# DavidPeicho/cuda-pathtracer

Measured on AMD Instinct MI355X. Metric: Msamples/sec at 1920x1080, 4 spp, indoor.obj, higher is better.
Workload: dtype f32

## Files before the change

### cuda-pathtracer_amd/csrc/pt_device.h

```cpp
#pragma once

#include <hip/hip_runtime.h>
#include <stdint.h>

#include "pt_round.h"

namespace ptamd {

struct f3 { float x, y, z; };

#define PT_DEV __device__ __forceinline__
#define PT_HD __host__ __device__ __forceinline__

PT_HD f3 mk3(float x, float y, float z) { f3 r; r.x = x; r.y = y; r.z = z; return r; }
PT_HD f3 mk3(float s) { return mk3(s, s, s); }
PT_HD f3 operator+(f3 a, f3 b) { return mk3(a.x + b.x, a.y + b.y, a.z + b.z); }
PT_HD f3 operator+(f3 a, float b) { return mk3(a.x + b, a.y + b, a.z + b); }
PT_HD f3 operator-(f3 a, f3 b) { return mk3(a.x - b.x, a.y - b.y, a.z - b.z); }
PT_HD f3 operator-(f3 a, float b) { return mk3(a.x - b, a.y - b, a.z - b); }
PT_HD f3 operator-(f3 a) { return mk3(-a.x, -a.y, -a.z); }
PT_HD f3 operator*(f3 a, f3 b) { return mk3(a.x * b.x, a.y * b.y, a.z * b.z); }
PT_HD f3 operator*(f3 a, float b) { return mk3(a.x * b, a.y * b, a.z * b); }
PT_HD f3 operator*(float b, f3 a) { return mk3(b * a.x, b * a.y, b * a.z); }
PT_HD f3 operator/(f3 a, f3 b) { return mk3(a.x / b.x, a.y / b.y, a.z / b.z); }
PT_HD f3 operator/(f3 a, float b) { return mk3(a.x / b, a.y / b, a.z / b); }
PT_HD f3 operator/(float b, f3 a) { return mk3(b / a.x, b / a.y, b / a.z); }
PT_HD float dot(f3 a, f3 b) { return a.x * b.x + a.y * b.y + a.z * b.z; }
PT_HD f3 cross(f3 a, f3 b) { return mk3(a.y * b.z - a.z * b.y, a.z * b.x - a.x * b.z, a.x * b.y - a.y * b.x); }
PT_DEV f3 normalize(f3 v) { float inv_len = 1.0f / __builtin_sqrtf(dot(v, v)); return v * inv_len; }

#ifndef PT_SHORT_MATH
#define PT_SHORT_MATH 1
#endif
PT_DEV float rcp_exact_in_range(float x)
{
  const float y0 = __builtin_amdgcn_rcpf(x);
  const float e0 = __builtin_fmaf(-x, y0, 1.0f);
  const float y1 = __builtin_fmaf(e0, y0, y0);
  const float r1 = __builtin_fmaf(-x, y1, 1.0f);
  const float q1 = __builtin_fmaf(r1, y1, y1);
  const float r2 = __builtin_fmaf(-x, q1, 1.0f);
  return __builtin_fmaf(r2, y1, q1);
}
PT_DEV float sqrt_exact_in_range(float x)
{
  float s = __builtin_amdgcn_sqrtf(x);
  const float sd = __uint_as_float(__float_as_uint(s) - 1u), su = __uint_as_float(__float_as_uint(s) + 1u);
  const float rd = __builtin_fmaf(-sd, s, x), ru = __builtin_fmaf(-su, s, x);
  s = rd <= 0.0f ? sd : s;
  s = ru > 0.0f ? su : s;
  return s;
}
PT_DEV bool wave_all(bool c) { return __builtin_amdgcn_ballot_w64(!c) == 0ull; }
PT_DEV f3 normalize_hot(f3 v)
{
  const float d = dot(v, v);
  float inv_len;
  if (PT_SHORT_MATH && wave_all(d >= 0x1p-96f && d < __builtin_inff())) inv_len = rcp_exact_in_range(sqrt_exact_in_range(d));
  else inv_len = 1.0f / __builtin_sqrtf(d);
  return v * inv_len;
}
PT_DEV float rcp_hot(float x)
{
  if (PT_SHORT_MATH && wave_all(x >= 0x1p-95f && x <= 0x1p125f)) return rcp_exact_in_range(x);
  return 1.0f / x;
}
PT_DEV float sqrt_checked(float x)
{
  if (PT_SHORT_MATH && wave_all(!(x < 0x1p-96f) || x == 0.0f)) return sqrt_exact_in_range(x);
  return __builtin_sqrtf(x);
}
PT_DEV float sqrt_hot(float x) { return PT_SHORT_MATH ? sqrt_exact_in_range(x) : __builtin_sqrtf(x); }
PT_DEV f3 reflect(f3 i, f3 n) { return i - (2.0f * n) * dot(n, i); }
PT_DEV f3 mix(f3 x, f3 y, float a) { return (x * (1.0f - a)) + y * a; }
PT_HD float clamp01(float f) { float m = f < 1.0f ? f : 1.0f; return 0.0f > m ? 0.0f : m; }

PT_DEV uint32_t f_as_u(float f) { return __float_as_uint(f); }
PT_DEV float u_as_f(uint32_t u) { return __uint_as_float(u); }


PT_DEV void pt_sincosf(float x, float& s, float& c)
{
  const float two_over_pi = 0x1.45f306p-1f;
  const float pio2_hi = 0x1.921fb6p+0f;
  const float pio2_lo = -0x1.777a5cp-25f;
  float k = __builtin_rintf(x * two_over_pi);
  float r = __builtin_fmaf(-k, pio2_hi, x);
  r = __builtin_fmaf(-k, pio2_lo, r);
  float r2 = r * r;
  float ps = __builtin_fmaf(__builtin_fmaf(-1.9515295891e-4f, r2, 8.3321608736e-3f), r2, -1.6666654611e-1f);
  float sn = __builtin_fmaf(r * r2, ps, r);
  float pc = __builtin_fmaf(__builtin_fmaf(2.443315711809948e-5f, r2, -1.388731625493765e-3f), r2, 4.166664568298827e-2f);
  float cs = __builtin_fmaf(r2 * r2, pc, __builtin_fmaf(-0.5f, r2, 1.0f));
  int q = (int)k & 3;
  float so = (q & 1) ? cs : sn;
  float co = (q & 1) ? sn : cs;
  if (q == 1 || q == 2) co = -co;
  if (q >= 2) so = -so;
  s = so;
  c = co;
}

__constant__ double kPowLog[9] = { 1.0 / 17.0, 1.0 / 15.0, 1.0 / 13.0, 1.0 / 11.0, 1.0 / 9.0, 1.0 / 7.0, 1.0 / 5.0, 1.0 / 3.0, 1.0 };
__constant__ double kPowExp[14] = { 1.0 / 6227020800.0, 1.0 / 479001600.0, 1.0 / 39916800.0, 1.0 / 3628800.0,
                                    1.0 / 362880.0, 1.0 / 40320.0, 1.0 / 5040.0, 1.0 / 720.0, 1.0 / 120.0,
                                    1.0 / 24.0, 1.0 / 6.0, 0.5, 1.0, 1.0 };

#ifndef __HIP_DEVICE_COMPILE__
static constexpr double kPowLogHost[9] = { 1.0 / 17.0, 1.0 / 15.0, 1.0 / 13.0, 1.0 / 11.0, 1.0 / 9.0, 1.0 / 7.0, 1.0 / 5.0, 1.0 / 3.0, 1.0 };
static constexpr double kPowExpHost[14] = { 1.0 / 6227020800.0, 1.0 / 479001600.0, 1.0 / 39916800.0, 1.0 / 3628800.0,
                                            1.0 / 362880.0, 1.0 / 40320.0, 1.0 / 5040.0, 1.0 / 720.0, 1.0 / 120.0,
                                            1.0 / 24.0, 1.0 / 6.0, 0.5, 1.0, 1.0 };
#define kPowLog kPowLogHost
#define kPowExp kPowExpHost
#define __double_as_longlong(x) __builtin_bit_cast(long long, (double)(x))
#define __longlong_as_double(x) __builtin_bit_cast(double, (long long)(x))
#endif

#ifdef __HIP_DEVICE_COMPILE__
__host__ __device__ __noinline__ float pt_powf(float xf, float yf)
#else
static __host__ __device__ __noinline__ float pt_powf(float xf, float yf)
#endif
{
  if (yf == 0.0f || xf == 1.0f) return 1.0f;
  if (xf != xf || yf != yf) return __builtin_nanf("");
  double x = (double)xf, y = (double)yf;
  bool negate = false;
  if (xf < 0.0f) {
    if (__builtin_floorf(yf) != yf) return __builtin_nanf("");
    float h = __builtin_fabsf(yf) * 0.5f;
    negate = __builtin_floorf(h) != h;
    x = -x;
  }
  double res;
  const double inf = __builtin_inf();
  if (x == 0.0) {
    res = y > 0.0 ? 0.0 : inf;
  } else if (x == inf) {
    res = y > 0.0 ? inf : 0.0;
  } else if (y == inf || y == -inf) {
    res = ((x > 1.0) == (y > 0.0)) ? inf : 0.0;
  } else {
    uint64_t b = (uint64_t)__double_as_longlong(x);
    int e = (int)((b >> 52) & 0x7ff) - 1023;
    double m = __longlong_as_double((long long)((b & 0x000fffffffffffffULL) | 0x3ff0000000000000ULL));
    if (m > 0x1.6a09e667f3bcdp+0) { m *= 0.5; e += 1; }
    double s = (m - 1.0) / (m + 1.0);
    double s2 = s * s;
    double p = kPowLog[0];
#pragma unroll
    for (int i = 1; i < 8; ++i) p = __builtin_fma(p, s2, kPowLog[i]);
    double lnm = 2.0 * s * __builtin_fma(p, s2, kPowLog[8]);
    double log2x = (double)e + lnm * 0x1.71547652b82fep+0;
    double z = y * log2x;
    if (z > 1100.0) {
      res = inf;
    } else if (z < -1100.0) {
      res = 0.0;
    } else {
      double n = __builtin_rint(z);
      double t = (z - n) * 0x1.62e42fefa39efp-1;
      double q = kPowExp[0];
#pragma unroll
      for (int i = 1; i < 14; ++i) q = __builtin_fma(q, t, kPowExp[i]);
      int ni = (int)n;
      int n1 = ni / 2, n2 = ni - n1;
      double s1 = __longlong_as_double((long long)((uint64_t)(n1 + 1023) << 52));
      double s2b = __longlong_as_double((long long)((uint64_t)(n2 + 1023) << 52));
      res = q * s1 * s2b;
    }
  }
  return (float)(negate ? -res : res);
}
#ifndef __HIP_DEVICE_COMPILE__
#undef kPowLog
#undef kPowExp
#undef __double_as_longlong
#undef __longlong_as_double
#endif

PT_HD uint32_t pt_f2u(float v)
{
  if (!(v > 0.0f)) return 0u;
  if (v >= 4294967296.0f) return 0xffffffffu;
  return (uint32_t)v;
}


PT_HD f3 uncharted_tonemap(f3 x)
{
  const float A = 0.15f, B = 0.50f, C = 0.10f, D = 0.20f, E = 0.02f, F = 0.30f;
  return ((x * (A * x + C * B) + D * E) / (x * (A * x + B) + D * F)) - E / F;
}

PT_HD f3 exposure(f3 color)
{
  const float exposure_bias = 2.0f;
  const f3 curr = uncharted_tonemap(exposure_bias * color);
  const f3 W = mk3(11.2f);
  const f3 white_scale = 1.0f / uncharted_tonemap(W);
  return curr * white_scale;
}

PT_HD f3 post_process(uint32_t id, f3 c)
{
  if (id == 1) {
    const float gray = (float)((double)c.x * 0.3 + (double)c.y * 0.59 + (double)c.z * 0.11);
    return mk3(gray, gray, gray);
  }
  if (id == 2)
    return mk3((float)((double)c.x * 0.393 + (double)c.y * 0.769 + (double)c.z * 0.189),
               (float)((double)c.x * 0.349 + (double)c.y * 0.686 + (double)c.z * 0.168),
               (float)((double)c.x * 0.272 + (double)c.y * 0.534 + (double)c.z * 0.131));
  if (id == 3)
    return mk3((float)(1.0 - (double)c.x), (float)(1.0 - (double)c.y), (float)(1.0 - (double)c.z));
  return c;
}

PT_HD uint32_t gamma_byte_exact(float x)
{
  return pt_f2u(pt_powf(x, 1.0f / 2.2f) * 255.0f) & 0xffu;
}
PT_HD uint32_t gamma_value_exact(float x) { return pt_f2u(pt_powf(x, 1.0f / 2.2f) * 255.0f); }

template <typename TablePtr>
PT_DEV uint32_t gamma_byte(float x, TablePtr T)
{
  if (!(x < T[256])) return gamma_byte_exact(x);
  if (!(x > 0.0f)) return 0u;
  const float est = __builtin_amdgcn_exp2f(__builtin_amdgcn_logf(x) * (1.0f / 2.2f)) * 255.0f;
  int k = (int)est;
  k = k < 0 ? 0 : (k > 255 ? 255 : k);
  k = x < T[k] ? k - 1 : k;
  k = x >= T[k + 1] ? k + 1 : k;
  return (uint32_t)k;
}

template <typename TablePtr>
PT_HD uint32_t output_pixel(f3 rad, uint32_t post_id, bool use_table, TablePtr T)
{
  rad = exposure(rad);
#ifdef __HIP_DEVICE_COMPILE__
  if (use_table) return gamma_byte(rad.x, T) | (gamma_byte(rad.y, T) << 8) | (gamma_byte(rad.z, T) << 16);
#endif
  const float g = 1.0f / 2.2f;
  rad = mk3(pt_powf(rad.x, g), pt_powf(rad.y, g), pt_powf(rad.z, g));
  rad = post_process(post_id, rad);
  return (pt_f2u(rad.x * 255.0f) & 0xffu) | ((pt_f2u(rad.y * 255.0f) & 0xffu) << 8) | ((pt_f2u(rad.z * 255.0f) & 0xffu) << 16);
}


struct Xorwow { uint32_t v0, v1, v2, v3, v4, d; };

PT_DEV uint32_t wang_hash(uint32_t a)
{
  a = (a ^ 61u) ^ (a >> 16);
  a = a + (a << 3);
  a = a ^ (a >> 4);
  a = a * 0x27d4eb2du;
  a = a ^ (a >> 15);
  return a;
}

PT_DEV void xorwow_init(Xorwow& st, uint32_t seed)
{
  uint32_t s0 = seed ^ 0xaad26b49u;
  uint32_t s1 = 0xf7dcefddu;
  uint32_t t0 = 1099087573u * s0;
  uint32_t t1 = 2591861531u * s1;
  st.v0 = 123456789u + t0;
  st.v1 = 362436069u ^ t0;
  st.v2 = 521288629u + t1;
  st.v3 = 88675123u ^ t1;
  st.v4 = 5783321u + t0;
  st.d = 6615241u + t1 + t0;
}

PT_HD float xorwow_uniform(Xorwow& st)
{
  uint32_t t = st.v0 ^ (st.v0 >> 2);
  st.v0 = st.v1; st.v1 = st.v2; st.v2 = st.v3; st.v3 = st.v4;
  st.v4 = (st.v4 ^ (st.v4 << 4)) ^ (t ^ (t << 1));
  st.d += 362437u;
  uint32_t x = st.v4 + st.d;
  return (float)x * 2.3283064e-10f + (2.3283064e-10f / 2.0f);
}


PT_HD float max3(f3 v) { return __builtin_fmaxf(v.x, __builtin_fmaxf(v.y, v.z)); }

template <class Rcp>
PT_HD bool miss_tail_iteration(f3 env, int max_bounces, f3& acc, f3& thr, uint32_t& bk, float& r1, Xorwow& rng, Rcp rcp)
{
  acc = acc + env * thr;
  const float pmax = max3(thr);
  if (r1 > pmax && (bk & 0xffffu) > 1u) return true;
  thr = thr * rcp(pmax);
  ++bk;
  if ((int)(bk & 0xffffu) >= max_bounces) return true;
  r1 = xorwow_uniform(rng);
  return false;
}

PT_HD bool miss_tail_is_closed(f3 thr) { return max3(thr) == 1.0f; }
PT_HD uint32_t miss_tail_count(uint32_t b, int max_bounces) { const int n = max_bounces - (int)b; return n > 1 ? (uint32_t)n : 1u; }
template <class Rcp>
PT_HD uint32_t miss_tail_finish(f3 env, int max_bounces, f3& acc, f3& thr, uint32_t& bk, float& r1, Xorwow& rng, Rcp rcp)
{
  uint32_t futile = 0;
  while (!miss_tail_is_closed(thr)) {
    if (miss_tail_iteration(env, max_bounces, acc, thr, bk, r1, rng, rcp)) return futile;
    ++futile;
  }
  const f3 e = env * thr;
  const uint32_t n = miss_tail_count(bk & 0xffffu, max_bounces);
  for (uint32_t i = 0; i < n; ++i) acc = acc + e;
  return futile + n - 1u;
}


struct TexDesc { int32_t w, h, nb_chan; uint32_t pad; uint64_t offset; };

#define PT_HEAD_STRIDE 64u
#ifndef PT_TILE_W_LOG2
#define PT_TILE_W_LOG2 3u
#endif
#define PT_TILE_W (1u << PT_TILE_W_LOG2)
#define PT_TILE_H (64u >> PT_TILE_W_LOG2)
struct KParams {
  const float4* nodes;
  const float4* tris_bvh;
  const float4* tris_brute;
  const float4* shade;
  const int4* materials;
  const float4* lights;
  const TexDesc* textures;
  const float* texels;
  const float4* cubemap;
  uint32_t cubemap_size;
  uint32_t n_faces, n_lights, n_nodes, n_bvh_tris;
  f3 cam_pos, cam_p0, cam_u, cam_v;
  float focus_dist, aperture;
  uint32_t width, height, row_begin, row_end;
  uint32_t hash_seed;
  float frame_nb_f;
  float frame_nb_inv;
  int32_t is_static;
  int32_t bounces;
  uint32_t post_id;
  float* tfb;
  uint32_t* surface;
  uint32_t tfb_row0;
  uint32_t tfb_reset;
  uint32_t surf_row0;
  unsigned long long* stats;
  unsigned long long* error_flag;
  union { uint32_t* tile_counter; uint32_t* adaptive; };
  uint32_t* tile_heads;
  uint32_t n_static;
  uint32_t tiles_x, n_tiles, tiles_per_ticket;
  uint32_t refill_min;
  uint32_t sample_count, frame_nb0;
  float* samples_out;
  float4* pool;
  uint32_t pool_lds_offset;
  uint32_t round_min, round_div;
  uint32_t round_div_m16;
  uint32_t walk_min;
  uint32_t small_det;
  uint32_t env_uniform;
  float env_r, env_g, env_b;
  const float* gamma_table;
  const float4* nodes4;
  uint32_t n_nodes4;
  uint32_t stack_lds_entries, stack_spill_entries;
  uint32_t ilv_ranks, ilv_rank, ilv_rows;
  uint32_t y_limit;
  uint32_t treelet_nodes;
  uint2* stack_spill;
  uint32_t walk_min4;
  uint32_t wide8;
  uint32_t far_table[16];
  uint32_t xcd_regions;
  uint32_t brute_walk;
  unsigned long long* timeline;
  uint32_t round_form;
  uint32_t round_defer;
};
#define PT_ROUND_GENERIC 1u
#define PT_ROUND_FLAT 2u
#define PT_ROUND_SKIP 4u
#define PT_ROUND_DEFER 8u
#define PT_ROUND_TIGHT 16u
inline bool round_form_tight(uint32_t round_form, uint32_t small_det, bool knob)
{
  const uint32_t needs = PT_ROUND_FLAT | PT_ROUND_SKIP | PT_ROUND_DEFER;
  return knob && small_det != 0u && (round_form & needs) == needs;
}
#define PT_SKIP_ENTRY_BYTES 32u

#define PT_RS_PLAIN 0
#define PT_RS_STATS 1
#define PT_RS_STAMPS 2
#define PT_RS_BRUTE 3
#define PT_RS_WIDE8 4
#define PT_RS_WIDE4Q 5
#define PT_RS_GENERIC 6
#define PT_RS_LIST 7
#define PT_RS_FLAT 8
#define PT_RS_FLAT_SKIP 9
#define PT_RS_PLAIN_SKIP 10
#define PT_RS_FLAT_SKIP_DEFER 11
#define PT_RS_PLAIN_SKIP_DEFER 12
#define PT_RS_STATS_DEFER 13
#define PT_RS_FLAT_SKIP_TIGHT 14
#define PT_RS_FORMS 15

struct RestartTraits {
  bool stats;
  bool stamps;
  bool brute;
  int wide;
  bool list;
  bool lean;
  bool flat;
  bool skip;
  bool defer;
  bool tight;
  int reports;
  bool resident, streamed, contracted;
};
constexpr RestartTraits kRestartForms[] = {
  { false, false, false, 0, false, true,  false, false, false, false, PT_RS_PLAIN,      true,  true,  true },
  { true,  false, false, 0, false, false, false, false, false, false, PT_RS_STATS,      true,  true,  false },
  { false, true,  false, 0, false, false, false, false, false, false, PT_RS_STAMPS,     true,  true,  false },
  { false, false, true,  0, false, false, false, false, false, false, PT_RS_BRUTE,      true,  true,  true },
  { false, false, false, 1, false, false, false, false, false, false, PT_RS_WIDE8,      false, true,  false },
  { false, false, false, 2, false, false, false, false, false, false, PT_RS_WIDE4Q,     false, true,  false },
  { false, false, false, 0, false, false, false, false, false, false, PT_RS_GENERIC,    true,  false, true },
  { false, false, false, 0, true,  false, false, false, false, false, PT_RS_LIST,       true,  true,  false },
  { false, false, false, 0, false, true,  true,  false, false, false, PT_RS_FLAT,       true,  false, false },
  { false, false, false, 0, false, true,  true,  true,  false, false, PT_RS_FLAT_SKIP,  true,  false, false },
  { false, false, false, 0, false, true,  false, true,  false, false, PT_RS_PLAIN_SKIP, true,  false, false },
  { false, false, false, 0, false, true,  true,  true,  true,  false, PT_RS_FLAT_SKIP,  true,  false, false },
  { false, false, false, 0, false, true,  false, true,  true,  false, PT_RS_PLAIN_SKIP, true,  false, false },
  { true,  false, false, 0, false, false, false, false, true,  false, PT_RS_STATS,      true,  false, false },
  { false, false, false, 0, false, true,  true,  true,  true,  true,  PT_RS_FLAT_SKIP,  true,  false, false },
};
static_assert(sizeof kRestartForms / sizeof kRestartForms[0] == PT_RS_FORMS, "one row per PT_RS_* number");
constexpr RestartTraits restart_traits(int variant) { return kRestartForms[variant]; }

inline bool restart_shipped_launch(const KParams& p)
{
  return p.is_static && p.pool_lds_offset && !p.xcd_regions && p.ilv_ranks <= 1u && !(p.round_form & PT_ROUND_GENERIC);
}

struct RestartForm { int variant; bool lds_resident; };
inline RestartForm restart_select(bool lds_resident, bool stats, bool list, bool contracted, const KParams* p)
{
  const auto full = [contracted](int variant) { return contracted ? PT_RS_PLAIN : variant; };
  if (list && !contracted) return { PT_RS_LIST, lds_resident };
  const bool defers = p && lds_resident && !contracted && (p->round_form & PT_ROUND_DEFER) && (p->round_form & PT_ROUND_SKIP) && !p->brute_walk && !p->timeline &&
                      restart_shipped_launch(*p);
  if (stats) return { defers ? PT_RS_STATS_DEFER : full(PT_RS_STATS), lds_resident };
  if (p && p->brute_walk) return { PT_RS_BRUTE, lds_resident };
  if (p && p->timeline) return { full(PT_RS_STAMPS), lds_resident };
  if (!lds_resident && p && p->wide8) return { full(p->wide8 == 2u ? PT_RS_WIDE4Q : PT_RS_WIDE8), false };
  if (!lds_resident) return { PT_RS_PLAIN, false };
  if (p && !restart_shipped_launch(*p)) return { PT_RS_GENERIC, true };
  if (defers && (p->round_form & PT_ROUND_FLAT) && (p->round_form & PT_ROUND_TIGHT)) return { PT_RS_FLAT_SKIP_TIGHT, true };
  if (defers) return { (p->round_form & PT_ROUND_FLAT) ? PT_RS_FLAT_SKIP_DEFER : PT_RS_PLAIN_SKIP_DEFER, true };
  if (p && (p->round_form & PT_ROUND_SKIP) && !contracted) return { (p->round_form & PT_ROUND_FLAT) ? PT_RS_FLAT_SKIP : PT_RS_PLAIN_SKIP, true };
  if (p && (p->round_form & PT_ROUND_FLAT)) return { full(PT_RS_FLAT), true };
  return { PT_RS_PLAIN, true };
}
#define PT_POOL_LDS_BYTES 2304u

struct Hit {
  f3 normal;
  f3 diffuse_col;
  float dist;
  float specular_col;
  float ior;
  int light;
  float emission;
};

}
```

### cuda-pathtracer_amd/csrc/pt_kernels.hip

```cpp
#include "pt_device.h"
#include "pt_launch.h"
#include "pt_adaptive.h"

#include <utility>

#if defined(PT_FMA_BUILD) || defined(PT_TIGHT_BUILD)
#define PT_SIDE_UNIT 1
#endif

#ifndef PT_SIDE_UNIT
#include "pt_denoise.h"
#endif

namespace ptamd {

#ifndef PT_TILE_THREADS
#define PT_TILE_THREADS 512
#endif
#ifndef PT_TILE_WAVES_PER_EU
#define PT_TILE_WAVES_PER_EU 6
#endif
#ifndef PT_SP_THREADS
#define PT_SP_THREADS 768
#endif
// ... 1596 lines not shown
      const bool any_leaf = __ballot(cur != PT_NONE && (cur & PT_LEAF_BIT)) != 0ull;
      if (PT_WAVE_ONE()) { cnt.cyc[1] += (unsigned long long)(tb1 - tb0); if (any_leaf) cnt.cyc[5]++; }
    }
    if (cur != PT_NONE && (cur & PT_LEAF_BIT)) {
      const uint32_t first = cur & 0xFFFFFFu, count = (cur >> 24) & 0x7Fu;
      constexpr uint32_t TS = 3u;
      const float4* t = tris + (size_t)first * TS;
      float4 r[9];
#pragma unroll
      for (uint32_t k = 0; k < 3u; ++k)
        if (k < count) { r[3 * k] = t[TS * k]; r[3 * k + 1] = t[TS * k + 1]; r[3 * k + 2] = t[TS * k + 2]; }
#pragma unroll
      for (uint32_t k = 0; k < 3u; ++k)
        if (k < count) {
          if (STATS) {
            const unsigned long long act = __ballot(1);
            if ((threadIdx.x & 63u) == (uint32_t)(__ffsll((long long)act) - 1)) ++cnt.wave_tri_iters;
          }
          mt_test<false>(r[3 * k], r[3 * k + 1], r[3 * k + 2], w.o, w.d, w.best, small_det);
        }
      if (STATS) cnt.tris += count < 3u ? count : 3u;
      if (count > 3u) walk_leaf<STATS>(tris, w, first + 3u, count - 3u, cnt.tris, cnt.wave_tri_iters, small_det, TS);
      cur = stack4_pop4(stk, sp, w.best.t);
    }
    if (STATS && PT_WAVE_ONE()) cnt.cyc[2] += (unsigned long long)(clock64() - tb1);
    if ((uint32_t)__popcll(__ballot(cur != PT_NONE)) < t_eff) break;
  }
  best = w.best;
}

PT_DEV bool region_tile(const KParams& p, uint32_t ticket, uint32_t& col, uint32_t& row, uint32_t& k)
{
  const uint32_t r = ticket & 7u, i = ticket >> 3;
  const uint32_t tiles_x = PT_KARG(p, tiles_x), tiles_y = PT_KARG(p, n_tiles) / tiles_x, count = PT_KARG(p, sample_count);
  const uint32_t rx = r & 3u, ry = r >> 2;
  const uint32_t x0 = rx * tiles_x / 4u, x1 = (rx + 1u) * tiles_x / 4u, y0 = ry * tiles_y / 2u, y1 = (ry + 1u) * tiles_y / 2u;
  const uint32_t w = x1 - x0, h = y1 - y0;
  const uint32_t j = i / count;
  if (j >= w * h) return false;
  k = i - j * count;
  const uint32_t strips = w / 8u, full = strips * 8u * h;
  if (j < full) {
    const uint32_t s = j / (8u * h), rem = j - s * 8u * h;
    row = y0 + rem / 8u;
    col = x0 + s * 8u + (rem & 7u);
  } else {
    const uint32_t rem = j - full, wl = w - strips * 8u;
    row = y0 + rem / wl;
    col = x0 + strips * 8u + rem % wl;
  }
  return true;
}

#define PT_STAMP(slot)                                                                                                   \
  do {                                                                                                                   \
    if (FORM.stamps) {                                                                                                   \
      unsigned long long* tl_ = PT_KARG(p, timeline);                            \
      if ((threadIdx.x & 63u) == 0u)                                                                                     \
        tl_[(size_t)(blockIdx.x * (THREADS / 64u) + (threadIdx.x >> 6)) * 4u + (slot)] = wall_clock64();                 \
    }                                                                                                                    \
  } while (0)

template <bool LDS_RESIDENT, int VARIANT>
__global__ void __launch_bounds__(LDS_RESIDENT ? PT_RS_THREADS : PT_RS4_THREADS, LDS_RESIDENT ? PT_RS_WAVES_PER_EU : PT_RS4_WAVES_PER_EU)
pt_megakernel_restart(PT_KERNEL_PARAMS)
{
  constexpr RestartTraits FORM = restart_traits(VARIANT);
  constexpr bool STATS = FORM.stats;
  constexpr uint32_t THREADS = LDS_RESIDENT ? PT_RS_THREADS : PT_RS4_THREADS;
  constexpr bool DEFER = LDS_RESIDENT && FORM.defer;
  constexpr bool TIGHT = DEFER && FORM.tight;
  static_assert(!FORM.tight || (FORM.defer && FORM.skip && FORM.lean && !FORM.stats && PT_ASM_LEAF), "the tight round is the flat deferring skip form's");
  constexpr uint32_t WALK_OVER = TIGHT ? 0xFFFFu : PT_END;
  constexpr bool SKIP = LDS_RESIDENT && FORM.skip;
  constexpr bool FLAT = LDS_RESIDENT && FORM.flat;
  constexpr bool LEAN = LDS_RESIDENT && FORM.lean;
  constexpr bool LIST = FORM.list;
  constexpr bool FIXED = LEAN || LIST;
  extern __shared__ float4 s_mem[];
  const float4* s_nodes;
  const float4* s_tris;
  PT_STAMP(0);
  stage_scene<2, LDS_RESIDENT, LDS_RESIDENT && !STATS, SKIP, TIGHT>(p, s_mem, s_nodes, s_tris);
  constexpr bool WIDE = !LDS_RESIDENT;

  const uint32_t lane = threadIdx.x & 63u;
  const uint32_t gwave = blockIdx.x * (THREADS / 64u) + (threadIdx.x >> 6);
  float4* slab = p.pool + (size_t)gwave * 192u;
  uint32_t* lds_pool = reinterpret_cast<uint32_t*>(reinterpret_cast<char*>(s_mem) + p.pool_lds_offset) + (threadIdx.x >> 6) * 576u;
  Stack4 stk;
  stk.top = s_mem;
  stk.top_n = WIDE ? p.treelet_nodes : 0u;
  constexpr uint32_t NODE_F4 = FORM.wide == 2 ? 4u : 8u;
  const uint32_t treelet_f4 = (WIDE && p.treelet_nodes) ? 8u * PT_TREELET_STRIDE : 0u;
  if (WIDE) {
    constexpr uint32_t PLANE = PT_TREELET_STRIDE * (8u / NODE_F4);
    for (uint32_t i = threadIdx.x; i < p.treelet_nodes * NODE_F4; i += blockDim.x) s_mem[(i % NODE_F4) * PLANE + i / NODE_F4] = p.nodes4[i];
    __syncthreads();
  }
  PT_STAMP(1);
  stk.lds = reinterpret_cast<uint2*>(s_mem + (size_t)treelet_f4) + (size_t)(threadIdx.x >> 6) * p.stack_lds_entries * 64u + lane;
  stk.spill = p.stack_spill + (size_t)gwave * p.stack_spill_entries * 64u + lane;
  stk.lds_entries = p.stack_lds_entries;
  uint32_t cur = PT_NONE, sp = 0;
  Counters cnt = {};
  uint32_t samples = 0;

  Path st;
  st.o = st.d = st.throughput = st.acc = mk3(0.f);
  st.rng.v0 = st.rng.v1 = st.rng.v2 = st.rng.v3 = st.rng.v4 = st.rng.d = 0;
  st.specular_col = 0.f; st.xy = 0; st.bk = 0;
  bool idle = true;
  bool walking = false;
  Best best;
  best.t = PT_MAX_DIST; best.u = best.v = 0.f; best.idx = PT_END;
  uint32_t node = WALK_OVER;
  uint32_t pool_rd = 64u, tile_x0 = 0, tile_y0 = 0, tile_k = 0;
  uint32_t tile_row_delta = 0;
  uint32_t tile = 0, tile_end = 0;
  uint32_t ticket = (!FIXED && PT_KARG(p, xcd_regions)) ? ((blockIdx.x >> 3) * (THREADS / 64u) + (threadIdx.x >> 6)) * 8u + (blockIdx.x & 7u) : gwave;
  ticket = (uint32_t)__builtin_amdgcn_readfirstlane((int)ticket);
  uint32_t reg_col = 0, reg_row = 0, reg_k = 0;
  uint32_t head = blockIdx.x & 7u, dry = 0;
  bool have_ticket = true, exhausted = false;
  uint32_t list_n = 0, list_chunks = 0, list_base = 0;
  if constexpr (LIST) {
    list_n = (uint32_t)__builtin_amdgcn_readfirstlane((int)*ad_active(p.adaptive, p.width * p.height));
    list_chunks = (list_n + 63u) >> 6;
  }
  for (;;) {
    long long tr0 = 0;
    if (STATS) tr0 = clock64();
    unsigned long long need = __ballot(idle);
    while (need) {
      if (pool_rd >= 64u) {
        if (exhausted) break;
        if (tile >= tile_end) {
          const uint32_t tiles_per_ticket = PT_KARG(p, tiles_per_ticket);
          uint32_t total;
          if constexpr (LIST) total = list_chunks * PT_KARG(p, sample_count);
          else total = PT_KARG(p, n_tiles) * PT_KARG(p, sample_count);
          for (;;) {
            if (!have_ticket) {
              uint32_t* heads = PT_KARG(p, tile_heads);
              uint32_t t = 0;
              if (lane == 0) t = atomicAdd(heads + head * PT_HEAD_STRIDE, 1u);
              t = (uint32_t)__builtin_amdgcn_readfirstlane((int)t);
              ticket = PT_KARG(p, n_static) + t * 8u + head;
            }
            have_ticket = false;
            if ((!FIXED && PT_KARG(p, xcd_regions)) ? region_tile(p, ticket, reg_col, reg_row, reg_k) : ((unsigned long long)ticket * tiles_per_ticket < total)) break;
            head = (head + 1u) & 7u;
            if (++dry == 8u) break;
          }
          if (dry == 8u) { exhausted = true; PT_STAMP(2); break; }
          if (!FIXED && PT_KARG(p, xcd_regions)) { tile = ticket; tile_end = ticket + 1u; }
          else {
            tile = ticket * tiles_per_ticket;
            tile_end = tile + tiles_per_ticket;
            if (tile_end > total) tile_end = total;
          }
        }
        if constexpr (LIST) {
          tile_k = tile / list_chunks;
          list_base = (tile - tile_k * list_chunks) * 64u;
        } else {
          const uint32_t n_tiles = PT_KARG(p, n_tiles), tiles_x = PT_KARG(p, tiles_x), row_begin = PT_KARG(p, row_begin);
          uint32_t local_y0;
          if (!FIXED && PT_KARG(p, xcd_regions)) {
            tile_k = reg_k; tile_x0 = reg_col * PT_TILE_W; local_y0 = reg_row * PT_TILE_H;
          } else {
            tile_k = tile / n_tiles;
            const uint32_t tl = tile - tile_k * n_tiles;
            tile_x0 = (tl % tiles_x) * PT_TILE_W;
            local_y0 = (tl / tiles_x) * PT_TILE_H;
          }
          const uint32_t ilv_ranks = LEAN ? 0u : PT_KARG(p, ilv_ranks);
          if (ilv_ranks > 1u) {
            const uint32_t ilv_rows = PT_KARG(p, ilv_rows);
            const uint32_t b = local_y0 / ilv_rows, within = local_y0 - b * ilv_rows;
            tile_y0 = (b * ilv_ranks + PT_KARG(p, ilv_rank)) * ilv_rows + within;
          } else {
            tile_y0 = row_begin + local_y0;
          }
          tile_row_delta = tile_y0 - (row_begin + local_y0);
        }
        ++tile;
        if constexpr (LIST) {
          const uint32_t i = list_base + lane;
          if (i < list_n) {
            const uint32_t n_px = p.width * p.height;
            const uint32_t px = ad_list(p.adaptive, n_px)[i];
            Path fresh;
            path_begin(p, px % p.width, px / p.width, fresh, tile_k, ad_counts(p.adaptive)[px] + 1u + tile_k);
            if (LDS_RESIDENT) pool_store_lds(lds_pool, lane, fresh);
            else pool_store(slab, lane, fresh);
          }
          if (!LDS_RESIDENT) asm volatile("s_waitcnt vmcnt(0)" ::: "memory");
        } else {
          const uint32_t x = tile_x0 + (lane & (PT_TILE_W - 1u)), y = tile_y0 + (lane >> PT_TILE_W_LOG2);
          if (x < p.width && y < p.y_limit) {
            Path fresh;
            path_begin(p, x, y, fresh, tile_k);
            if (LEAN || p.pool_lds_offset) pool_store_lds(lds_pool, lane, fresh);
            else pool_store(slab, lane, fresh);
          }
          if (!LEAN && !p.pool_lds_offset) asm volatile("s_waitcnt vmcnt(0)" ::: "memory");
        }
        pool_rd = 0u;
      }
      const uint32_t rank = __builtin_amdgcn_mbcnt_hi((uint32_t)(need >> 32), __builtin_amdgcn_mbcnt_lo((uint32_t)need, 0u));
      const uint32_t avail = 64u - pool_rd;
      if constexpr (LIST) {
        const uint32_t i = list_base + pool_rd + rank;
        if (idle && rank < avail && i < list_n) {
          if (LDS_RESIDENT) pool_load_lds(lds_pool, pool_rd + rank, st);
          else pool_load(slab, pool_rd + rank, st);
          st.throughput = mk3(1.0f);
          st.acc = mk3(0.0f);
          st.specular_col = 0.0f;
          st.xy = (i % p.width) | ((i / p.width) << 16);
          st.bk = tile_k << 16;
          idle = false;
          walking = false;
        }
      } else if (idle && rank < avail) {
        const uint32_t e = pool_rd + rank;
        const uint32_t x = tile_x0 + (e & (PT_TILE_W - 1u)), y = tile_y0 + (e >> PT_TILE_W_LOG2);
        if (x < p.width && y < p.y_limit) {
          if (LEAN || p.pool_lds_offset) pool_load_lds(lds_pool, e, st);
          else pool_load(slab, e, st);
          st.throughput = mk3(1.0f);
          st.acc = mk3(0.0f);
          st.specular_col = 0.0f;
          st.xy = x | ((y - tile_row_delta) << 16);
          st.bk = tile_k << 16;
          idle = false;
          walking = false;
        }
      }
      const uint32_t wanted = (uint32_t)__popcll(need);
      pool_rd += wanted < avail ? wanted : avail;
      need = __ballot(idle);
    }
    if (__ballot(!idle) == 0ull) break;
    long long tr1 = 0;
    if (STATS) { tr1 = clock64(); if (PT_WAVE_ONE()) cnt.cyc[0] += (unsigned long long)(tr1 - tr0); }

    if (!idle) {
      if (!walking) {
        best.t = PT_MAX_DIST; best.u = 0.f; best.v = 0.f; best.idx = PT_END;
        if (TIGHT) node = PT_WALK_FRESH;
        else if (SKIP) node = reinterpret_cast<const uint32_t*>(s_mem)[(st.d.x < 0.f ? 1u : 0u) | (st.d.y < 0.f ? 2u : 0u) | (st.d.z < 0.f ? 4u : 0u)];
        else node = p.n_nodes ? 0u : PT_END;
        cur = p.n_nodes4 ? 0u : PT_NONE;
        sp = 0u;
        walking = true;
        if (STATS) cnt.rays++;
      }
      if (FORM.brute) {
        for (uint32_t i = 0; i < p.n_bvh_tris; ++i) mt_test<false>(s_tris[i * 3u], s_tris[i * 3u + 1u], s_tris[i * 3u + 2u], st.o, st.d, best, false);
        if (STATS) cnt.tris += p.n_bvh_tris;
        node = PT_END;
      } else if (WIDE) {
        traverse_round4<STATS, FORM.wide>(p, p.nodes4, s_tris, stk, st.o, st.d, best, cur, sp, p.round_min, p.round_div, p.round_div_m16, p.walk_min4, p.small_det != 0u, cnt);
        node = cur == PT_NONE ? PT_END : 0u;
      } else if constexpr (TIGHT) {
        traverse_round_tight(s_nodes, s_tris, reinterpret_cast<const uint32_t*>(s_mem), p.n_nodes, st.o, st.d, best, node, p.round_min, (p.round_defer >> 8) == 0xFFu ? PT_LEAF_DEFER_AUTO : p.round_defer >> 8,
                             p.round_div, p.round_div_m16, p.walk_min);
      } else {
        traverse_round<STATS, LDS_RESIDENT, DEFER>(s_nodes, s_tris, p.n_nodes, st.o, st.d, best, node, DEFER ? p.round_defer : p.round_min, p.round_div, p.round_div_m16, p.walk_min, p.small_det != 0u, cnt);
      }
      if (STATS) {
        if (lane == (uint32_t)(__ffsll((long long)__ballot(1)) - 1)) cnt.fetch_events++;
        if (node == WALK_OVER) cnt.fetch_rays++;
      }
      if (node == WALK_OVER) {
        long long tl0 = 0;
        if (STATS) tl0 = clock64();
        const float r1 = path_pre<FIXED>(p, st);
        Nearest n;
        n.t = best.t; n.u = best.u; n.v = best.v; n.idx = best.idx;
        n = nearest_lights(p, st.o, st.d, n);
        walking = false;
        long long tl1 = 0;
        if (STATS) { asm volatile("" : "+v"(n.t), "+v"(n.idx)); tl1 = clock64(); if (PT_WAVE_ONE()) cnt.cyc[3] += (unsigned long long)(tl1 - tl0); }
        if (path_post<STATS, FIXED, FLAT>(p, st, r1, n, cnt)) {
          path_finish_sample(p, st);
          idle = true;
          if (STATS) samples++;
        }
        if (STATS) { const long long tl2 = clock64(); if (PT_WAVE_ONE()) cnt.cyc[9] += (unsigned long long)(tl2 - tl1); }
      }
    }
    if (STATS) {
      const long long tr3 = clock64();
      if (PT_WAVE_ONE()) cnt.cyc[4] += (unsigned long long)(tr3 - tr0);
    }
  }
  PT_STAMP(3);
  flush_counters<STATS>(p, cnt, samples);
}


template <bool LDS_RESIDENT, bool STATS>
__global__ void __launch_bounds__(PT_BW_THREADS, PT_BW_WAVES_PER_EU) pt_megakernel_blockwise(PT_KERNEL_PARAMS)
{
  constexpr uint32_t NW = PT_BW_THREADS / 64u;
  constexpr uint32_t NE = NW * 8u;
  constexpr uint32_t EPL = (NE + 63u) / 64u;
  static_assert(NW % 4u == 0 && NE <= 128u, "workgroup must be 4k waves, at most 16");
  extern __shared__ float4 s_mem[];
  const float4* s_nodes;
  const float4* s_tris;
  stage_scene<2, LDS_RESIDENT>(p, s_mem, s_nodes, s_tris);
  float4* pool = s_mem + (LDS_RESIDENT ? (p.n_nodes * 4u + p.n_bvh_tris * 3u) : 0u);
  uint32_t* s_cnt = reinterpret_cast<uint32_t*>(pool + PT_BW_THREADS * 2u);
  uint32_t* s_head = s_cnt + 128;
  uint32_t* s_ticket = s_cnt + 129;

  const uint32_t tid = threadIdx.x, lane = tid & 63u, wave = tid >> 6;
  Counters cnt = {};
  uint32_t samples = 0;
  uint32_t ticket = blockIdx.x;

  for (;;) {
    if (ticket >= p.n_tiles) break;
    const uint32_t sx = (ticket % p.tiles_x) * 32u, sy = p.row_begin + (ticket / p.tiles_x) * (NW * 2u);
    const uint32_t x = sx + (wave & 3u) * 8u + (lane & 7u);
    const uint32_t y = sy + (wave >> 2) * 8u + (lane >> 3);
    const bool active = x < p.width && y < p.row_end;
    Path st;
    bool live = active;
    if (active) path_begin(p, x, y, st);
    else { st.o = st.d = st.throughput = st.acc = mk3(0.f); st.xy = 0; st.bk = 0; st.specular_col = 0.f;
           st.rng.v0 = st.rng.v1 = st.rng.v2 = st.rng.v3 = st.rng.v4 = st.rng.d = 0; }

    if (live) live = !path_step<2, STATS>(p, s_nodes, s_tris, st, cnt);

    for (;;) {
      const uint32_t oct = (st.d.x < 0.f ? 1u : 0u) | (st.d.y < 0.f ? 2u : 0u) | (st.d.z < 0.f ? 4u : 0u);
      uint32_t rank = 0, my_count = 0;
#pragma unroll
      for (uint32_t o = 0; o < 8u; ++o) {
        const unsigned long long m = __ballot(live && oct == o);
        const uint32_t c = (uint32_t)__popcll(m);
        if (oct == o) rank = __builtin_amdgcn_mbcnt_hi((uint32_t)(m >> 32), __builtin_amdgcn_mbcnt_lo((uint32_t)m, 0u));
        if (lane == o) my_count = c;
      }
      if (lane < 8u) s_cnt[lane * NW + wave] = my_count;
      if (tid == 0) *s_head = 0u;
      __syncthreads();
      uint32_t e0 = 0, e1 = 0;
      if (lane * EPL < NE) e0 = s_cnt[lane * EPL];
      if (EPL == 2u && lane * EPL + 1u < NE) e1 = s_cnt[lane * EPL + 1u];
      uint32_t incl = e0 + e1;
#pragma unroll
      for (int off = 1; off < 64; off <<= 1) {
        const uint32_t up = __shfl_up(incl, off, 64);
        if ((int)lane >= off) incl += up;
      }
      const uint32_t n_live = __shfl(incl, 63, 64);
      if (n_live == 0) break;
      const uint32_t excl = incl - (e0 + e1);
      const uint32_t entry = oct * NW + wave;
      uint32_t base = __shfl(excl, (int)(entry / EPL), 64);
      if (EPL == 2u) { const uint32_t first = __shfl(e0, (int)(entry / EPL), 64); if (entry & 1u) base += first; }
      const uint32_t slot = base + rank;
      float r1 = 0.f;
      if (live) {
        r1 = path_pre(p, st);
        pool[slot * 2u + 0u] = make_float4(st.d.x, st.d.y, st.d.z, st.o.x);
        pool[slot * 2u + 1u] = make_float4(st.o.y, st.o.z, 0.f, 0.f);
      }
      __syncthreads();

      {
        Walk w;
        w.node = PT_END; w.oct = 0; w.link_off = 8u;
        w.o = w.d = w.inv = w.noi = mk3(0.f);
        w.best.t = PT_MAX_DIST; w.best.u = w.best.v = 0.f; w.best.idx = PT_END;
        bool have = false;
        uint32_t my_ray = 0;
        bool pool_empty = false;
        for (;;) {
          const unsigned long long idle_mask = __ballot(!have);
          const uint32_t n_idle = (uint32_t)__popcll(idle_mask);
          if (!pool_empty && (n_idle >= PT_BW_FETCH_MIN || idle_mask == ~0ull)) {
            uint32_t head = 0;
            if (lane == 0) head = atomicAdd(s_head, n_idle);
            head = (uint32_t)__builtin_amdgcn_readfirstlane((int)head);
            const uint32_t r = head + __builtin_amdgcn_mbcnt_hi((uint32_t)(idle_mask >> 32),
                                                                __builtin_amdgcn_mbcnt_lo((uint32_t)idle_mask, 0u));
            if (!have && r < n_live) {
              const float4 ra = pool[r * 2u + 0u], rb = pool[r * 2u + 1u];
              walk_init(w, mk3(ra.w, rb.x, rb.y), mk3(ra.x, ra.y, ra.z), p.n_nodes);
              have = true;
              my_ray = r;
              if (STATS) cnt.rays++;
            }
            if (head + n_idle >= n_live) pool_empty = true;
          }
          if (__ballot(have) == 0ull) break;
          if (have) {
            uint32_t leaf_first, leaf_count;
            walk_to_leaf<STATS>(s_nodes, w, leaf_first, leaf_count, cnt.nodes, cnt.wave_node_iters);
            if (leaf_count != 0u) {
              walk_leaf<STATS>(s_tris, w, leaf_first, leaf_count, cnt.tris, cnt.wave_tri_iters);
            } else if (w.node == PT_END) {
              pool[my_ray * 2u + 0u] = make_float4(w.best.t, w.best.u, w.best.v, u_as_f(w.best.idx));
              have = false;
            }
          }
        }
      }
      __syncthreads();
      if (live) {
        const float4 h = pool[slot * 2u + 0u];
        Nearest n;
        n.t = h.x; n.u = h.y; n.v = h.z; n.idx = f_as_u(h.w);
        n = nearest_lights(p, st.o, st.d, n);
        live = !path_post<STATS>(p, st, r1, n, cnt);
      }
    }

    if (active) { path_finish(p, st); if (STATS) samples++; }
    __syncthreads();
    if (tid == 0) *s_ticket = atomicAdd(p.tile_counter, 1u);
    __syncthreads();
    ticket = *s_ticket;
  }
  flush_counters<STATS>(p, cnt, samples);
}


template <bool LDS_RESIDENT, bool STATS>
__global__ void __launch_bounds__(PT_SP_THREADS, PT_SP_WAVES_PER_EU) pt_megakernel_split(PT_KERNEL_PARAMS)
{
  constexpr uint32_t NW = PT_SP_THREADS / 64u, NS = PT_SP_SHADERS, NT = NW - NS;
  static_assert(NS >= 1 && NT >= 1, "need at least one shader wave and one traverser wave");
  extern __shared__ float4 s_mem[];
  const float4* s_nodes;
  const float4* s_tris;
  stage_scene<2, LDS_RESIDENT, LDS_RESIDENT && !STATS>(p, s_mem, s_nodes, s_tris);
  float4* rays = s_mem + (LDS_RESIDENT ? (p.n_nodes * 4u + p.n_bvh_tris * 3u) : 0u);
  uint32_t* word = reinterpret_cast<uint32_t*>(rays + NS * 64u * 2u);
  uint32_t* done = word + NS;
  uint32_t* fin = done + NS;
  const uint32_t tid = threadIdx.x, lane = tid & 63u, wave = tid >> 6;
  if (tid < NS) { word[tid] = 0u; done[tid] = 0u; }
  if (tid == 0) *fin = 0u;
  __syncthreads();

  Counters cnt = {};
  uint32_t samples = 0;
  const uint32_t spin_limit = 1u << 26;

  if (wave < NS) {
    float4* my_rays = rays + wave * 128u;
    const uint32_t total = p.n_tiles * p.sample_count;
    uint32_t ticket = blockIdx.x * NS + wave;
    bool failed = false;
    while (ticket < total && !failed) {
      const uint32_t k = ticket / p.n_tiles, tl = ticket - k * p.n_tiles;
      const uint32_t x = (tl % p.tiles_x) * PT_TILE_W + (lane & (PT_TILE_W - 1u));
      const uint32_t y = p.row_begin + (tl / p.tiles_x) * PT_TILE_H + (lane >> PT_TILE_W_LOG2);
      const bool active = x < p.width && y < p.row_end;
      Path st;
      if (active) path_begin(p, x, y, st, k);
      else { st.o = st.d = st.throughput = st.acc = mk3(0.f); st.xy = 0; st.bk = 0; st.specular_col = 0.f;
             st.rng.v0 = st.rng.v1 = st.rng.v2 = st.rng.v3 = st.rng.v4 = st.rng.d = 0; }
      bool live = active;
      for (;;) {
        const unsigned long long m = __ballot(live);
        const uint32_t n = (uint32_t)__popcll(m);
        if (n == 0) break;
        const uint32_t slot = __builtin_amdgcn_mbcnt_hi((uint32_t)(m >> 32), __builtin_amdgcn_mbcnt_lo((uint32_t)m, 0u));
        float r1 = 0.f;
        if (live) {
          r1 = path_pre(p, st);
          my_rays[slot * 2u + 0u] = make_float4(st.d.x, st.d.y, st.d.z, st.o.x);
          my_rays[slot * 2u + 1u] = make_float4(st.o.y, st.o.z, 0.f, 0.f);
          if (STATS) cnt.rays++;
        }
        __builtin_amdgcn_fence(__ATOMIC_RELEASE, "workgroup");
        if (lane == 0) {
          __hip_atomic_store(&done[wave], 0u, __ATOMIC_RELAXED, __HIP_MEMORY_SCOPE_WORKGROUP);
          __hip_atomic_store(&word[wave], n << 16, __ATOMIC_RELEASE, __HIP_MEMORY_SCOPE_WORKGROUP);
        }
        uint32_t spins = 0, d = 0;
        do {
          d = __hip_atomic_load(&done[wave], __ATOMIC_ACQUIRE, __HIP_MEMORY_SCOPE_WORKGROUP);
          d = (uint32_t)__builtin_amdgcn_readfirstlane((int)d);
          if (d != n) __builtin_amdgcn_s_sleep(2);
        } while (d != n && ++spins < spin_limit);
        if (d != n) { failed = true; break; }
        if (lane == 0) __hip_atomic_store(&word[wave], 0u, __ATOMIC_RELAXED, __HIP_MEMORY_SCOPE_WORKGROUP);
        __builtin_amdgcn_fence(__ATOMIC_ACQUIRE, "workgroup");
        if (live) {
          const float4 h = my_rays[slot * 2u + 0u];
          Nearest nr;
          nr.t = h.x; nr.u = h.y; nr.v = h.z; nr.idx = f_as_u(h.w);
          nr = nearest_lights(p, st.o, st.d, nr);
          live = !path_post<STATS>(p, st, r1, nr, cnt);
        }
      }
      if (failed) break;
      if (active) {
        if (p.sample_count > 1u) path_finish_sample(p, st);
        else path_finish(p, st);
        if (STATS) samples++;
      }
      uint32_t t = 0;
      if (lane == 0) t = atomicAdd(p.tile_counter, 1u);
      ticket = (uint32_t)__builtin_amdgcn_readfirstlane((int)t);
    }
    if (failed && lane == 0) atomicAdd(p.error_flag, 1ull);
    if (lane == 0) __hip_atomic_fetch_add(fin, 1u, __ATOMIC_RELEASE, __HIP_MEMORY_SCOPE_WORKGROUP);
  } else {
    Walk w;
    w.node = PT_END; w.oct = 0; w.link_off = 8u;
    w.o = w.d = w.inv = w.noi = mk3(0.f);
    w.best.t = PT_MAX_DIST; w.best.u = w.best.v = 0.f; w.best.idx = PT_END;
    const uint32_t lds_nodes = (uint32_t)(uintptr_t)s_nodes;
    bool have = false;
    uint32_t my_slot = 0;
    uint32_t scan = (wave - NS) % NS, idle_spins = 0;
    for (;;) {
      const unsigned long long idle_mask = __ballot(!have);
      const uint32_t n_idle = (uint32_t)__popcll(idle_mask);
      if (n_idle >= PT_SP_FETCH_MIN || idle_mask == ~0ull) {
        uint32_t got = 0, base = 0, b = scan;
        for (uint32_t tries = 0; tries < NS && got == 0; ++tries) {
          uint32_t wd = __hip_atomic_load(&word[b], __ATOMIC_RELAXED, __HIP_MEMORY_SCOPE_WORKGROUP);
          wd = (uint32_t)__builtin_amdgcn_readfirstlane((int)wd);
          if ((wd & 0xffffu) < (wd >> 16)) {
            uint32_t old = 0;
            if (lane == 0) old = __hip_atomic_fetch_add(&word[b], n_idle, __ATOMIC_ACQUIRE, __HIP_MEMORY_SCOPE_WORKGROUP);
            old = (uint32_t)__builtin_amdgcn_readfirstlane((int)old);
            const uint32_t on = old >> 16, oc = old & 0xffffu;
            if (oc < on) { base = oc; got = on - oc < n_idle ? on - oc : n_idle; }
          }
          if (got == 0) b = b + 1u == NS ? 0u : b + 1u;
        }
        scan = b;
        if (got) {
          __builtin_amdgcn_fence(__ATOMIC_ACQUIRE, "workgroup");
          const uint32_t rank = __builtin_amdgcn_mbcnt_hi((uint32_t)(idle_mask >> 32),
                                                          __builtin_amdgcn_mbcnt_lo((uint32_t)idle_mask, 0u));
          if (!have && rank < got) {
            const uint32_t r = base + rank;
            const float4 ra = rays[(b * 64u + r) * 2u + 0u], rb = rays[(b * 64u + r) * 2u + 1u];
            walk_init(w, mk3(ra.w, rb.x, rb.y), mk3(ra.x, ra.y, ra.z), p.n_nodes, LDS_RESIDENT && !STATS);
            have = true;
            my_slot = (b << 8) | r;
          }
          idle_spins = 0;
          if (STATS && lane == 0) { cnt.fetch_events++; cnt.fetch_rays += got; }
        } else if (idle_mask == ~0ull) {
          uint32_t f = __hip_atomic_load(fin, __ATOMIC_ACQUIRE, __HIP_MEMORY_SCOPE_WORKGROUP);
          f = (uint32_t)__builtin_amdgcn_readfirstlane((int)f);
          if (f == NS || ++idle_spins >= spin_limit) break;
          __builtin_amdgcn_s_sleep(2);
          continue;
        }
      }
      if (have) {
        uint32_t leaf_first, leaf_count;
        if (LDS_RESIDENT && !STATS) walk_to_leaf_lds(lds_nodes, w, leaf_first, leaf_count);
        else walk_to_leaf<STATS>(s_nodes, w, leaf_first, leaf_count, cnt.nodes, cnt.wave_node_iters);
        if (leaf_count != 0u) {
          walk_leaf<STATS>(s_tris, w, leaf_first, leaf_count, cnt.tris, cnt.wave_tri_iters);
        } else if (w.node == PT_END) {
          const uint32_t b = my_slot >> 8, r = my_slot & 0xffu;
          rays[(b * 64u + r) * 2u + 0u] = make_float4(w.best.t, w.best.u, w.best.v, u_as_f(w.best.idx));
          __builtin_amdgcn_fence(__ATOMIC_RELEASE, "workgroup");
          __hip_atomic_fetch_add(&done[b], 1u, __ATOMIC_RELEASE, __HIP_MEMORY_SCOPE_WORKGROUP);
          have = false;
        }
      }
    }
  }
  flush_counters<STATS>(p, cnt, samples);
}


__global__ void __launch_bounds__(320) pt_build_gamma_table(float* T)
{
  const uint32_t j = threadIdx.x;
  if (j > 256u) return;
  if (j == 0u) { T[0] = 0.0f; T[257] = 0.0f; return; }
  uint32_t lo = 0u, hi = 0x7F800000u;
  while (hi - lo > 1u) {
    const uint32_t mid = lo + (hi - lo) / 2u;
    if (gamma_value_exact(u_as_f(mid)) >= j) hi = mid; else lo = mid;
  }
  T[j] = u_as_f(hi);
}

__global__ void __launch_bounds__(256) pt_gamma_selftest(const float* T, uint32_t first, uint32_t count, unsigned long long* out)
{
  __shared__ float s_T[258];
  for (uint32_t i = threadIdx.x; i < 258u; i += 256u) s_T[i] = T[i];
  __syncthreads();
  unsigned long long bad = 0;
  for (uint32_t i = blockIdx.x * 256u + threadIdx.x; i < count; i += gridDim.x * 256u) {
// ... 493 lines not shown
```

Measured before the change: 14930.

## Add tight restart megakernel variant with compact per-path state and magic-number tile division

Adds a specialized restart megakernel for the flat/skip/defer/tight round form. Each path's pixel is encoded as a single byte offset into the sample output instead of separate coordinates, and tile indices are decoded with precomputed reciprocal multiplies rather than integer division. The goal is to cut per-path register state and integer ALU work in the refill loop. The variant is only chosen when the 32-bit offset cannot overflow, and it is compiled only under PT_TIGHT_BUILD.

```diff
diff --git a/cuda-pathtracer_amd/csrc/pt_device.h b/cuda-pathtracer_amd/csrc/pt_device.h
--- a/cuda-pathtracer_amd/csrc/pt_device.h
+++ b/cuda-pathtracer_amd/csrc/pt_device.h
@@ -4,6 +4,7 @@
 #include <stdint.h>
 
 #include "pt_round.h"
+#include "pt_tight_tiles.h"
 
 namespace ptamd {
 
@@ -469,7 +470,7 @@
   if (!lds_resident && p && p->wide8) return { full(p->wide8 == 2u ? PT_RS_WIDE4Q : PT_RS_WIDE8), false };
   if (!lds_resident) return { PT_RS_PLAIN, false };
   if (p && !restart_shipped_launch(*p)) return { PT_RS_GENERIC, true };
-  if (defers && (p->round_form & PT_ROUND_FLAT) && (p->round_form & PT_ROUND_TIGHT)) return { PT_RS_FLAT_SKIP_TIGHT, true };
+  if (defers && (p->round_form & PT_ROUND_FLAT) && (p->round_form & PT_ROUND_TIGHT) && tight_slab_fits(p->sample_count, p->row_end - p->row_begin, p->width)) return { PT_RS_FLAT_SKIP_TIGHT, true };
   if (defers) return { (p->round_form & PT_ROUND_FLAT) ? PT_RS_FLAT_SKIP_DEFER : PT_RS_PLAIN_SKIP_DEFER, true };
   if (p && (p->round_form & PT_ROUND_SKIP) && !contracted) return { (p->round_form & PT_ROUND_FLAT) ? PT_RS_FLAT_SKIP : PT_RS_PLAIN_SKIP, true };
   if (p && (p->round_form & PT_ROUND_FLAT)) return { full(PT_RS_FLAT), true };
diff --git a/cuda-pathtracer_amd/csrc/pt_kernels.hip b/cuda-pathtracer_amd/csrc/pt_kernels.hip
--- a/cuda-pathtracer_amd/csrc/pt_kernels.hip
+++ b/cuda-pathtracer_amd/csrc/pt_kernels.hip
@@ -1922,6 +1922,10 @@
   flush_counters<STATS>(p, cnt, samples);
 }
 
+#ifdef PT_TIGHT_BUILD
+#include "pt_tight_body.h"
+#endif
+
 
 template <bool LDS_RESIDENT, bool STATS>
 __global__ void __launch_bounds__(PT_BW_THREADS, PT_BW_WAVES_PER_EU) pt_megakernel_blockwise(PT_KERNEL_PARAMS)
diff --git a/cuda-pathtracer_amd/csrc/pt_tight_body.h b/cuda-pathtracer_amd/csrc/pt_tight_body.h
--- /dev/null
+++ b/cuda-pathtracer_amd/csrc/pt_tight_body.h
@@ -0,0 +1,127 @@
+#pragma once
+
+static_assert(PT_TILE_W == PT_TT_TILE && PT_TILE_H == PT_TT_TILE, "pt_tight_tiles.h states the tile as 8 x 8");
+
+PT_DEV void tight_park(const KParams& p, uint32_t offset, f3 acc)
+{
+  float* sp = reinterpret_cast<float*>(reinterpret_cast<char*>(PT_KARG(p, samples_out)) + offset);
+  sp[0] = clamp01(acc.x); sp[1] = clamp01(acc.y); sp[2] = clamp01(acc.z);
+}
+
+#define PT_TIGHT_IDLE 0xFFFFFFFFu
+
+PT_DEV void tight_take(const uint32_t* lds_pool, uint32_t e, uint32_t offset, Path& st)
+{
+  pool_load_lds(lds_pool, e, st);
+  st.throughput = mk3(1.0f);
+  st.acc = mk3(0.0f);
+  st.specular_col = 0.0f;
+  st.xy = offset;
+  st.bk = 0u;
+}
+
+template <>
+__global__ void __launch_bounds__(PT_RS_THREADS, PT_RS_WAVES_PER_EU)
+pt_megakernel_restart<true, PT_RS_FLAT_SKIP_TIGHT>(PT_KERNEL_PARAMS)
+{
+  static_assert(PT_ASM_LEAF, "the tight round's leaf phase is the hand-written one");
+  extern __shared__ float4 s_mem[];
+  const float4* s_nodes;
+  const float4* s_tris;
+  stage_scene<2, true, true, true, true>(p, s_mem, s_nodes, s_tris);
+
+  const uint32_t lane = threadIdx.x & 63u;
+  const uint32_t gwave = blockIdx.x * (PT_RS_THREADS / 64u) + (threadIdx.x >> 6);
+  uint32_t* lds_pool = reinterpret_cast<uint32_t*>(reinterpret_cast<char*>(s_mem) + p.pool_lds_offset) + (threadIdx.x >> 6) * 576u;
+
+  Path st;
+  st.o = st.d = st.throughput = st.acc = mk3(0.f);
+  st.rng.v0 = st.rng.v1 = st.rng.v2 = st.rng.v3 = st.rng.v4 = st.rng.d = 0;
+  st.specular_col = 0.f; st.bk = 0;
+  st.xy = PT_TIGHT_IDLE;
+  Best best;
+  best.t = PT_MAX_DIST; best.u = best.v = 0.f; best.idx = PT_END;
+  uint32_t node = 0xFFFFu;
+  uint32_t pool_rd = 64u, tile_offset = 0, tile_width12 = 0, tile_lim = 0;
+  uint32_t tile = 0, tile_end = 0;
+  uint32_t ticket = (uint32_t)__builtin_amdgcn_readfirstlane((int)gwave);
+  uint32_t head = blockIdx.x & 7u, dry = 0;
+  uint32_t have_ticket = 1u;
+  const uint32_t m_tiles = (uint32_t)__builtin_amdgcn_readfirstlane((int)tight_div_magic(PT_KARG(p, n_tiles)));
+  const uint32_t m_x = (uint32_t)__builtin_amdgcn_readfirstlane((int)tight_div_magic(PT_KARG(p, tiles_x)));
+  for (;;) {
+    unsigned long long need = __ballot(st.xy == PT_TIGHT_IDLE);
+    while (need) {
+      if (__builtin_expect(pool_rd >= 64u, 0)) {
+        if (dry == 8u) break;
+        if (tile >= tile_end) {
+          const uint32_t tiles_per_ticket = PT_KARG(p, tiles_per_ticket);
+          const uint32_t total = PT_KARG(p, n_tiles) * PT_KARG(p, sample_count);
+          for (;;) {
+            if (!have_ticket) {
+              uint32_t* heads = PT_KARG(p, tile_heads);
+              uint32_t t = 0;
+              if (lane == 0) t = atomicAdd(heads + head * PT_HEAD_STRIDE, 1u);
+              t = (uint32_t)__builtin_amdgcn_readfirstlane((int)t);
+              ticket = PT_KARG(p, n_static) + t * 8u + head;
+            }
+            have_ticket = 0u;
+            if ((unsigned long long)ticket * tiles_per_ticket < total) break;
+            head = (head + 1u) & 7u;
+            if (++dry == 8u) break;
+          }
+          if (dry == 8u) break;
+          tile = ticket * tiles_per_ticket;
+          tile_end = tile + tiles_per_ticket;
+          if (tile_end > total) tile_end = total;
+        }
+        const uint32_t n_tiles = PT_KARG(p, n_tiles), tiles_x = PT_KARG(p, tiles_x), row_begin = PT_KARG(p, row_begin);
+        const TightTile at = tight_tile_at(tile, n_tiles, m_tiles, tiles_x, m_x);
+        const uint32_t tile_k = at.k, local_y0 = at.y0;
+        const uint32_t tile_x0 = at.x0, tile_y0 = row_begin + local_y0;
+        const uint32_t width = PT_KARG(p, width);
+        tile_width12 = width * 12u;
+        tile_offset = tight_tile_slot(tile_k, PT_KARG(p, row_end) - row_begin, local_y0, width, tile_x0) * 12u;
+        tile_lim = tight_tile_lim(width, p.y_limit, tile_x0, tile_y0);
+        ++tile;
+        const uint32_t x = tile_x0 + (lane & (PT_TILE_W - 1u)), y = tile_y0 + (lane >> PT_TILE_W_LOG2);
+        if (x < width && y < p.y_limit) {
+          Path fresh;
+          path_begin(p, x, y, fresh, tile_k);
+          pool_store_lds(lds_pool, lane, fresh);
+        }
+        pool_rd = 0u;
+      }
+      const uint32_t rank = __builtin_amdgcn_mbcnt_hi((uint32_t)(need >> 32), __builtin_amdgcn_mbcnt_lo((uint32_t)need, 0u));
+      const uint32_t avail = 64u - pool_rd;
+      if (st.xy == PT_TIGHT_IDLE && rank < avail) {
+        const uint32_t e = pool_rd + rank;
+        if (tight_entry_inside(tile_lim, e)) tight_take(lds_pool, e, tight_entry_offset(tile_offset, tile_width12, e), st);
+      }
+      const uint32_t wanted = (uint32_t)__popcll(need);
+      pool_rd += wanted < avail ? wanted : avail;
+      need = __ballot(st.xy == PT_TIGHT_IDLE);
+    }
+    if (dry == 8u && __ballot(st.xy != PT_TIGHT_IDLE) == 0ull) break;
+
+    if (st.xy != PT_TIGHT_IDLE) {
+      if (node == 0xFFFFu) {
+        best.t = PT_MAX_DIST; best.u = 0.f; best.v = 0.f; best.idx = PT_END;
+        node = PT_WALK_FRESH;
+      }
+      traverse_round_tight(s_nodes, s_tris, reinterpret_cast<const uint32_t*>(s_mem), p.n_nodes, st.o, st.d, best, node, p.round_min, (p.round_defer >> 8) == 0xFFu ? PT_LEAF_DEFER_AUTO : p.round_defer >> 8,
+                           p.round_div, p.round_div_m16, p.walk_min);
+      if (node == 0xFFFFu) {
+        const float r1 = path_pre<true>(p, st);
+        Nearest n;
+        n.t = best.t; n.u = best.u; n.v = best.v; n.idx = best.idx;
+        n = nearest_lights(p, st.o, st.d, n);
+        Counters cnt = {};
+        if (path_post<false, true, true>(p, st, r1, n, cnt)) {
+          tight_park(p, st.xy, st.acc);
+          st.xy = PT_TIGHT_IDLE;
+        }
+      }
+    }
+  }
+}
diff --git a/cuda-pathtracer_amd/csrc/pt_tight_tiles.h b/cuda-pathtracer_amd/csrc/pt_tight_tiles.h
--- /dev/null
+++ b/cuda-pathtracer_amd/csrc/pt_tight_tiles.h
@@ -0,0 +1,63 @@
+#pragma once
+#include <stdint.h>
+
+#if defined(__HIPCC__)
+#define PT_TT_HD __host__ __device__ __forceinline__
+#else
+#define PT_TT_HD inline
+#endif
+
+namespace ptamd {
+
+#define PT_TT_TILE 8u
+
+PT_TT_HD bool tight_slab_fits(uint32_t frames, uint32_t rows, uint32_t width)
+{
+  const unsigned long long a = (unsigned long long)frames * rows;
+  if (a == 0ull || width == 0u) return true;
+  return a <= (0x100000000ull / 12ull) / width;
+}
+
+PT_TT_HD uint32_t tight_tile_slot(uint32_t k, uint32_t rows, uint32_t local_y0, uint32_t width, uint32_t x0)
+{
+  return (k * rows + local_y0) * width + x0;
+}
+PT_TT_HD uint32_t tight_entry_offset(uint32_t tile_offset, uint32_t width12, uint32_t e)
+{
+  return tile_offset + (e >> 3) * width12 + (e & (PT_TT_TILE - 1u)) * 12u;
+}
+
+PT_TT_HD uint32_t tight_div_magic(uint32_t d) { return 0xFFFFFFFFu / (d ? d : 1u); }
+PT_TT_HD uint32_t tight_div(uint32_t n, uint32_t d, uint32_t m, uint32_t& rem)
+{
+  uint32_t q = (uint32_t)(((unsigned long long)n * m) >> 32);
+  uint32_t r = n - q * d;
+  if (r >= d) { r -= d; ++q; }
+  rem = r;
+  return q;
+}
+
+struct TightTile { uint32_t k, x0, y0; };
+
+PT_TT_HD TightTile tight_tile_at(uint32_t tile, uint32_t n_tiles, uint32_t m_tiles, uint32_t tiles_x, uint32_t m_x)
+{
+  TightTile t;
+  uint32_t tl, col;
+  t.k = tight_div(tile, n_tiles, m_tiles, tl);
+  t.y0 = tight_div(tl, tiles_x, m_x, col) * PT_TT_TILE;
+  t.x0 = col * PT_TT_TILE;
+  return t;
+}
+
+#define PT_TT_WHOLE (PT_TT_TILE | (PT_TT_TILE << 8))
+PT_TT_HD uint32_t tight_tile_lim(uint32_t width, uint32_t y_limit, uint32_t x0, uint32_t y0)
+{
+  const uint32_t in_x = width - x0, in_y = y_limit - y0;
+  return (in_x < PT_TT_TILE ? in_x : PT_TT_TILE) | ((in_y < PT_TT_TILE ? in_y : PT_TT_TILE) << 8);
+}
+PT_TT_HD bool tight_entry_inside(uint32_t lim, uint32_t e)
+{
+  return (e & (PT_TT_TILE - 1u)) < (lim & 0xFFu) && (e >> 3) < (lim >> 8);
+}
+
+}
```

After: 15250, median of 6. 1.02x the previous value.
